# VIDILabs/instantvnr

Measured on AMD Instinct MI355X. Metric: fps at 1024^2 on 1024^3 volume, higher is better.
Workload: dtype f16

## Files before the change

### instantvnr_amd/csrc/grid_device.h

```cpp
#pragma once

#include "network.h"

namespace vnr {

typedef _Float16 half_t;
typedef _Float16 half2_t __attribute__((ext_vector_type(2)));
typedef _Float16 half4_t __attribute__((ext_vector_type(4)));
typedef _Float16 half8_t __attribute__((ext_vector_type(8)));
typedef float float2_t __attribute__((ext_vector_type(2)));
typedef float float4_t __attribute__((ext_vector_type(4)));
typedef float float8_t __attribute__((ext_vector_type(8)));
typedef float f32x16 __attribute__((ext_vector_type(16)));
typedef uint32_t uint4_t __attribute__((ext_vector_type(4)));

struct CornerSetup {
  float w[3];
  uint32_t g[3];
};

__device__ __forceinline__ CornerSetup level_setup(const LevelInfo& lv, uint32_t interpolation, float x, float y, float z)
{
  CornerSetup c;
  const float in[3] = {x, y, z};
#pragma unroll
  for (int d = 0; d < 3; ++d) {
    float p = __builtin_fmaf(in[d], lv.scale, 0.5f);
    const float t = __builtin_floorf(p);
    c.g[d] = (uint32_t)(int32_t)t;
    p -= t;
    c.w[d] = p;
  }
  if (interpolation == 1) {
    asm volatile("" ::: "memory");
#pragma unroll
    for (int d = 0; d < 3; ++d) c.w[d] = c.w[d] * c.w[d] * (3.0f - 2.0f * c.w[d]);
  }
  return c;
}

__device__ __forceinline__ uint32_t level_index(const LevelInfo& lv, uint32_t px, uint32_t py, uint32_t pz)
{
  if (lv.hashed == 1u) {
    return (px ^ (py * 2654435761u) ^ (pz * 805459861u)) & (lv.size - 1u);
  }
  if (lv.hashed >= 2u) {
    uint32_t idx = px;
    if (lv.hashed >= 3u) idx += py * lv.resolution;
    if (lv.hashed >= 4u) idx += pz * (lv.resolution * lv.resolution);
    return idx % lv.size;
  }
  uint32_t idx = px + py * lv.resolution + pz * (lv.resolution * lv.resolution);
  if (idx >= lv.size) {
    idx -= lv.size;
    if (idx >= lv.size) idx %= lv.size;
  }
  return idx;
}

__device__ __forceinline__ float corner_weight(const CornerSetup& c, int corner)
{
  const float wx = (corner & 1) ? c.w[0] : 1.0f - c.w[0];
  const float wy = (corner & 2) ? c.w[1] : 1.0f - c.w[1];
  const float wz = (corner & 4) ? c.w[2] : 1.0f - c.w[2];
  return (wx * wy) * wz;
}

template <int F> struct FeatVec;
template <> struct FeatVec<1> { typedef half_t type; };
template <> struct FeatVec<2> { typedef half2_t type; };
template <> struct FeatVec<4> { typedef half4_t type; };
template <> struct FeatVec<8> { typedef half8_t type; };

template <int F>
__device__ __forceinline__ void encode_level(const LevelInfo& lv, uint32_t interpolation, const half_t* __restrict__ table,
                                             float x, float y, float z, half_t* out)
{
  typedef typename FeatVec<F>::type vec_t;
  const CornerSetup c = level_setup(lv, interpolation, x, y, z);
  const vec_t* __restrict__ base = (const vec_t*)(table + (size_t)lv.offset * F);
  vec_t v[8];
#pragma unroll
  for (int corner = 0; corner < 8; ++corner) {
    const uint32_t idx = level_index(lv, c.g[0] + (corner & 1), c.g[1] + ((corner >> 1) & 1), c.g[2] + ((corner >> 2) & 1));
    v[corner] = base[idx];
  }
  half_t acc[F];
#pragma unroll
  for (int f = 0; f < F; ++f) acc[f] = (half_t)0.0f;
#pragma unroll
  for (int corner = 0; corner < 8; ++corner) {
    const float w = corner_weight(c, corner);
    const half_t* d = (const half_t*)&v[corner];
#pragma unroll
    for (int f = 0; f < F; ++f) {
      float prod = w * (float)d[f];
      if (F == 1) asm volatile("" : "+v"(prod));
      acc[f] = acc[f] + (half_t)prod;
    }
  }
#pragma unroll
  for (int f = 0; f < F; ++f) out[f] = acc[f];
}

typedef __amdgpu_buffer_rsrc_t table_rsrc_t;

#ifndef VNR_HASH_QUAD
#define VNR_HASH_QUAD 1
#endif

__device__ __forceinline__ table_rsrc_t make_table_rsrc(const void* base, uint32_t bytes)
{
  return __builtin_amdgcn_make_buffer_rsrc(const_cast<void*>(base), 0, (int)bytes, 0x00020000);
}

template <int F> struct RawFeat;
template <> struct RawFeat<1> {
  typedef unsigned short raw_t;
  static __device__ __forceinline__ raw_t load(table_rsrc_t r, uint32_t voff, uint32_t soff) { return __builtin_amdgcn_raw_buffer_load_b16(r, voff, soff, 0); }
};
template <> struct RawFeat<2> {
  typedef uint32_t raw_t;
  static __device__ __forceinline__ raw_t load(table_rsrc_t r, uint32_t voff, uint32_t soff) { return __builtin_amdgcn_raw_buffer_load_b32(r, voff, soff, 0); }
};
template <> struct RawFeat<4> {
  typedef uint32_t raw_t __attribute__((ext_vector_type(2)));
  static __device__ __forceinline__ raw_t load(table_rsrc_t r, uint32_t voff, uint32_t soff) { return __builtin_amdgcn_raw_buffer_load_b64(r, voff, soff, 0); }
};
template <> struct RawFeat<8> {
  typedef uint4_t raw_t;
  static __device__ __forceinline__ raw_t load(table_rsrc_t r, uint32_t voff, uint32_t soff) { return __builtin_amdgcn_raw_buffer_load_b128(r, voff, soff, 0); }
};

template <int F> struct PairFeat { static constexpr bool enabled = false; };
template <> struct PairFeat<2> {
  static constexpr bool enabled = true;
  typedef uint32_t pair_t __attribute__((ext_vector_type(2)));
  static __device__ __forceinline__ pair_t load(table_rsrc_t r, uint32_t voff, uint32_t soff) { return __builtin_amdgcn_raw_buffer_load_b64(r, voff, soff, 0); }
  static __device__ __forceinline__ uint32_t lo(pair_t p) { return p.x; }
  static __device__ __forceinline__ uint32_t hi(pair_t p) { return p.y; }
};
template <> struct PairFeat<4> {
  static constexpr bool enabled = true;
  typedef uint4_t pair_t;
  typedef uint32_t half_pair_t __attribute__((ext_vector_type(2)));
  static __device__ __forceinline__ pair_t load(table_rsrc_t r, uint32_t voff, uint32_t soff) { return __builtin_amdgcn_raw_buffer_load_b128(r, voff, soff, 0); }
  static __device__ __forceinline__ half_pair_t lo(pair_t p) { return half_pair_t{p.x, p.y}; }
  static __device__ __forceinline__ half_pair_t hi(pair_t p) { return half_pair_t{p.z, p.w}; }
};

typedef uint32_t uint8x32_t __attribute__((ext_vector_type(8)));
__device__ __noinline__ uint8x32_t level_indices_exact(const LevelInfo lv, uint32_t g0, uint32_t g1, uint32_t g2)
{
  uint8x32_t idx;
#pragma unroll
  for (int corner = 0; corner < 8; ++corner)
    idx[corner] = level_index(lv, g0 + (corner & 1), g1 + ((corner >> 1) & 1), g2 + ((corner >> 2) & 1));
  return idx;
}

template <int F, bool GENERAL = false>
__device__ __forceinline__ void gather_corners(const LevelInfo& lv, const CornerSetup& c, table_rsrc_t rsrc,
                                               typename RawFeat<F>::raw_t (&v)[8])
{
  constexpr uint32_t kBytes = (uint32_t)(F * 2);
  const uint32_t soff = lv.offset * kBytes;
  if (GENERAL && lv.hashed >= 2u) {
    const uint8x32_t idx = level_indices_exact(lv, c.g[0], c.g[1], c.g[2]);
#pragma unroll
    for (int corner = 0; corner < 8; ++corner) v[corner] = RawFeat<F>::load(rsrc, idx[corner] * kBytes, soff);
  } else if (lv.hashed) {
    const uint32_t mask = lv.size - 1u;
    const uint32_t hy0 = c.g[1] * 2654435761u, hy1 = hy0 + 2654435761u;
    const uint32_t hz0 = c.g[2] * 805459861u, hz1 = hz0 + 805459861u;
    const uint32_t x0 = c.g[0], x1 = c.g[0] + 1u;
    const uint32_t yz[4] = {hy0 ^ hz0, hy1 ^ hz0, hy0 ^ hz1, hy1 ^ hz1};
    constexpr uint32_t kGroupMask = (F == 2 && VNR_HASH_QUAD) ? 3u : PairFeat<F>::enabled ? 1u : 0u;
    if (kGroupMask && mask < kGroupMask) {
      const uint8x32_t idx = level_indices_exact(lv, c.g[0], c.g[1], c.g[2]);
#pragma unroll
      for (int corner = 0; corner < 8; ++corner) v[corner] = RawFeat<F>::load(rsrc, idx[corner] * kBytes, soff);
      return;
    }
#if VNR_HASH_QUAD
    if constexpr (F == 2) {
      const uint32_t m = (x0 & 1u) ? 3u : 1u;
      const bool far_x = (x0 & 3u) == 3u;
      uint32_t i1[4];
#pragma unroll
      for (int q = 0; q < 4; ++q) {
        const uint32_t i0 = (x0 ^ yz[q]) & mask;
        i1[q] = (x1 ^ yz[q]) & mask;
        const uint4_t g = __builtin_amdgcn_raw_buffer_load_b128(rsrc, (i0 & ~3u) * kBytes, soff, 0);
        const uint32_t k = i0 & 3u, k2 = k ^ m;
        const uint32_t a0 = (k & 1u) ? g.y : g.x, a1 = (k & 1u) ? g.w : g.z;
        const uint32_t b0 = (k & 1u) ? g.x : g.y, b1 = (k & 1u) ? g.z : g.w;
        v[2 * q] = (k & 2u) ? a1 : a0;
        v[2 * q + 1] = (k2 & 2u) ? b1 : b0;
      }
      if (far_x) {
#pragma unroll
        for (int q = 0; q < 4; ++q) v[2 * q + 1] = RawFeat<F>::load(rsrc, i1[q] * kBytes, soff);
      }
    } else
#endif
    if constexpr (PairFeat<F>::enabled) {
      const bool odd_x = (x0 & 1u) != 0u;
      uint32_t i1[4];
#pragma unroll
      for (int q = 0; q < 4; ++q) {
        const uint32_t i0 = (x0 ^ yz[q]) & mask;
        i1[q] = (x1 ^ yz[q]) & mask;
        const auto pr = PairFeat<F>::load(rsrc, (i0 & ~1u) * kBytes, soff);
        const bool up = (i0 & 1u) != 0u;
        v[2 * q] = up ? PairFeat<F>::hi(pr) : PairFeat<F>::lo(pr);
        v[2 * q + 1] = up ? PairFeat<F>::lo(pr) : PairFeat<F>::hi(pr);
      }
      if (odd_x) {
#pragma unroll
        for (int q = 0; q < 4; ++q) v[2 * q + 1] = RawFeat<F>::load(rsrc, i1[q] * kBytes, soff);
      }
    } else {
#pragma unroll
      for (int corner = 0; corner < 8; ++corner)
        v[corner] = RawFeat<F>::load(rsrc, ((((corner & 1) ? x1 : x0) ^ yz[corner >> 1]) & mask) * kBytes, soff);
    }
  } else {
    const uint32_t res = lv.resolution, res2 = lv.res2;
    const uint32_t base = c.g[0] + __umul24(c.g[1], res) + __umul24(c.g[2], res2);
    const bool bad = (c.g[0] > res) | (c.g[1] > res) | (c.g[2] > res) | (base + 1u + res + res2 >= lv.size);
    if (__builtin_amdgcn_ballot_w64(bad) != 0ull) {
      const uint8x32_t idx = level_indices_exact(lv, c.g[0], c.g[1], c.g[2]);
#pragma unroll
      for (int corner = 0; corner < 8; ++corner) v[corner] = RawFeat<F>::load(rsrc, idx[corner] * kBytes, soff);
    } else if constexpr (PairFeat<F>::enabled) {
#pragma unroll
      for (int q = 0; q < 4; ++q) {
        const uint32_t idx = base + ((q & 1) ? res : 0u) + ((q & 2) ? res2 : 0u);
        const auto pr = PairFeat<F>::load(rsrc, idx * kBytes, soff);
        v[2 * q] = PairFeat<F>::lo(pr);
        v[2 * q + 1] = PairFeat<F>::hi(pr);
      }
    } else {
#pragma unroll
      for (int corner = 0; corner < 8; ++corner) {
        const uint32_t idx = base + ((corner & 1) ? 1u : 0u) + ((corner & 2) ? res : 0u) + ((corner & 4) ? res2 : 0u);
        v[corner] = RawFeat<F>::load(rsrc, idx * kBytes, soff);
      }
    }
  }
}

template <int F>
__device__ __forceinline__ bool gather_corners_brick(const LevelInfo& lv, const CornerSetup& c, const uint8_t* __restrict__ image,
                                                     typename RawFeat<F>::raw_t (&v)[8])
{
  typedef typename RawFeat<F>::raw_t raw_t;
  if constexpr (F == 2) {
    typedef typename PairFeat<F>::pair_t pair_t;
    const uint32_t res = lv.resolution;
    const bool bad = (c.g[0] >= res) | (c.g[1] >= res) | (c.g[2] >= res);
    if (__builtin_amdgcn_ballot_w64(bad) != 0ull) return false;
    const uint32_t nbx = lv.pad1, nby = (res >> 1) + 1u;
    const uint32_t bx = (c.g[0] * 9363u) >> 16;
    const uint32_t wx = c.g[0] - 7u * bx, wy = c.g[1] & 1u, wz = c.g[2] & 1u;
    const uint32_t brick = __umul24(__umul24(c.g[2] >> 1, nby) + (c.g[1] >> 1), nbx) + bx;
    const uint32_t e0 = brick * 32u + ((wz << 4) | (wy << 3) | wx);
    const uint32_t dy = wy ? nbx * 32u - 8u : 8u;
    const uint32_t dz = wz ? nbx * nby * 32u - 16u : 16u;
    const uint8_t* base = image + (size_t)(lv.brick - 1u) * 128u;
#pragma unroll
    for (int q = 0; q < 4; ++q) {
      const uint32_t e = e0 + ((q & 1) ? dy : 0u) + ((q & 2) ? dz : 0u);
      const pair_t pr = *(const pair_t*)(base + (size_t)e * 4u);
      v[2 * q] = PairFeat<F>::lo(pr);
      v[2 * q + 1] = PairFeat<F>::hi(pr);
    }
    return true;
  }
  constexpr uint32_t LX = BrickShape<F>::lx, LY = BrickShape<F>::ly, LZ = BrickShape<F>::lz;
  constexpr uint32_t MX = (1u << LX) - 1u, MY = (1u << LY) - 1u, MZ = (1u << LZ) - 1u;
  constexpr uint32_t E = 1u << (LX + LY + LZ);
  constexpr uint32_t kBytes = (uint32_t)(F * 2);
  static_assert(E * kBytes == 128, "a brick is one 128-byte line");
  const uint32_t res = lv.resolution;
  const bool bad = (c.g[0] >= res) | (c.g[1] >= res) | (c.g[2] >= res);
  if (__builtin_amdgcn_ballot_w64(bad) != 0ull) return false;
  const uint32_t nbx = (res >> LX) + 1u, nby = (res >> LY) + 1u;
  const uint32_t wx = c.g[0] & MX, wy = c.g[1] & MY, wz = c.g[2] & MZ;
  const uint32_t brick = __umul24(__umul24(c.g[2] >> LZ, nby) + (c.g[1] >> LY), nbx) + (c.g[0] >> LX);
  const uint32_t e0 = brick * E + ((wz << (LX + LY)) | (wy << LX) | wx);
  const uint32_t dx = wx == MX ? E - MX : 1u;
  const uint32_t dy = wy == MY ? nbx * E - (MY << LX) : 1u << LX;
  const uint32_t dz = wz == MZ ? nbx * nby * E - (MZ << (LX + LY)) : 1u << (LX + LY);
  const uint8_t* base = image + (size_t)(lv.brick - 1u) * 128u;
  if constexpr (PairFeat<F>::enabled) {
    typedef typename PairFeat<F>::pair_t pair_t;
#pragma unroll
    for (int q = 0; q < 4; ++q) {
      const uint32_t e = e0 + ((q & 1) ? dy : 0u) + ((q & 2) ? dz : 0u);
      const pair_t pr = *(const pair_t*)(base + (size_t)e * kBytes);
      v[2 * q] = PairFeat<F>::lo(pr);
      v[2 * q + 1] = PairFeat<F>::hi(pr);
    }
    if (wx == MX) {
#pragma unroll
      for (int q = 0; q < 4; ++q) {
        const uint32_t e = e0 + ((q & 1) ? dy : 0u) + ((q & 2) ? dz : 0u) + dx;
        v[2 * q + 1] = *(const raw_t*)(base + (size_t)e * kBytes);
      }
    }
  } else {
#pragma unroll
    for (int corner = 0; corner < 8; ++corner) {
      const uint32_t e = e0 + ((corner & 1) ? dx : 0u) + ((corner & 2) ? dy : 0u) + ((corner & 4) ? dz : 0u);
      v[corner] = *(const raw_t*)(base + (size_t)e * kBytes);
    }
  }
  return true;
}

__device__ __forceinline__ half2_t weighted_pair(float w, uint32_t pair)
{
  float lo, hi;
  asm("v_fma_mix_f32 %0, %1, %2, 0 op_sel_hi:[1,0,0]" : "=v"(lo) : "v"(pair), "v"(w));
  asm("v_fma_mix_f32 %0, %1, %2, 0 op_sel:[1,0,0] op_sel_hi:[1,0,0]" : "=v"(hi) : "v"(pair), "v"(w));
  return __builtin_convertvector(float2_t{lo, hi}, half2_t);
}

template <int F>
__device__ __forceinline__ void blend_level(const float (&wd)[3], const typename FeatVec<F>::type (&v)[8], half_t* out)
{
  const float wx0 = 1.0f - wd[0], wx1 = wd[0], wy0 = 1.0f - wd[1], wy1 = wd[1], wz0 = 1.0f - wd[2], wz1 = wd[2];
  const float wxy[4] = {wx0 * wy0, wx1 * wy0, wx0 * wy1, wx1 * wy1};
  if constexpr (F == 1) {
    half_t acc = (half_t)0.0f;
#pragma unroll
    for (int corner = 0; corner < 8; ++corner) {
      float prod = (wxy[corner & 3] * ((corner & 4) ? wz1 : wz0)) * (float)v[corner];
      asm volatile("" : "+v"(prod));
      acc = acc + (half_t)prod;
    }
    out[0] = acc;
  } else {
    typedef uint32_t words_t __attribute__((ext_vector_type(F / 2)));
    half2_t acc[F / 2];
#pragma unroll
    for (int q = 0; q < F / 2; ++q) acc[q] = half2_t{(half_t)0.0f, (half_t)0.0f};
#pragma unroll
    for (int corner = 0; corner < 8; ++corner) {
      const float w = wxy[corner & 3] * ((corner & 4) ? wz1 : wz0);
      const words_t words = __builtin_bit_cast(words_t, v[corner]);
#pragma unroll
      for (int q = 0; q < F / 2; ++q) {
        uint32_t word;
        if constexpr (F == 2) word = __builtin_bit_cast(uint32_t, words); else word = words[q];
        acc[q] = acc[q] + weighted_pair(w, word);
      }
    }
#pragma unroll
    for (int q = 0; q < F / 2; ++q) { out[2 * q] = acc[q].x; out[2 * q + 1] = acc[q].y; }
  }
}

template <int F>
__device__ __forceinline__ typename RawFeat<F>::raw_t quantize_raw(typename RawFeat<F>::raw_t raw, float qt)
{
  typedef typename FeatVec<F>::type vec_t;
  vec_t v = __builtin_bit_cast(vec_t, raw);
  if constexpr (F == 1) {
    if (fabsf((float)v) < qt) v = (half_t)0.0f;
  } else {
#pragma unroll
    for (int f = 0; f < F; ++f) if (fabsf((float)v[f]) < qt) v[f] = (half_t)0.0f;
  }
  return __builtin_bit_cast(typename RawFeat<F>::raw_t, v);
}

template <int F, bool GENERAL = false>
__device__ __forceinline__ void encode_level_fast(const LevelInfo& lv, uint32_t interpolation, table_rsrc_t rsrc, const uint8_t* image,
                                                  float x, float y, float z, half_t* out, float quantize_threshold = 0.0f)
{
  typedef typename RawFeat<F>::raw_t raw_t;
  const CornerSetup c = level_setup(lv, interpolation, x, y, z);
  if (GENERAL && interpolation == 2u) {
    const raw_t one = RawFeat<F>::load(rsrc, level_index(lv, c.g[0], c.g[1], c.g[2]) * (uint32_t)(F * 2), lv.offset * (uint32_t)(F * 2));
    const typename FeatVec<F>::type vv = __builtin_bit_cast(typename FeatVec<F>::type, one);
    if constexpr (F == 1) out[0] = vv;
    else {
#pragma unroll
      for (int f = 0; f < F; ++f) out[f] = vv[f];
    }
    return;
  }
  raw_t v[8];
  if (lv.brick == 0u || !gather_corners_brick<F>(lv, c, image, v)) gather_corners<F, GENERAL>(lv, c, rsrc, v);
  if (GENERAL && quantize_threshold > 0.0f) {
#pragma unroll
    for (int corner = 0; corner < 8; ++corner) v[corner] = quantize_raw<F>(v[corner], quantize_threshold);
  }
  if constexpr (F >= 2) {
    typename FeatVec<F>::type vv[8];
#pragma unroll
    for (int corner = 0; corner < 8; ++corner) vv[corner] = __builtin_bit_cast(typename FeatVec<F>::type, v[corner]);
    blend_level<F>(c.w, vv, out);
    return;
  }
  const float wx0 = 1.0f - c.w[0], wx1 = c.w[0], wy0 = 1.0f - c.w[1], wy1 = c.w[1], wz0 = 1.0f - c.w[2], wz1 = c.w[2];
  const float wxy[4] = {wx0 * wy0, wx1 * wy0, wx0 * wy1, wx1 * wy1};
  half_t acc[F];
#pragma unroll
  for (int f = 0; f < F; ++f) acc[f] = (half_t)0.0f;
#pragma unroll
  for (int corner = 0; corner < 8; ++corner) {
    const float w = wxy[corner & 3] * ((corner & 4) ? wz1 : wz0);
    const half_t* d = (const half_t*)&v[corner];
#pragma unroll
    for (int f = 0; f < F; ++f) {
      float prod = w * (float)d[f];
      if (F == 1) asm volatile("" : "+v"(prod));
      acc[f] = acc[f] + (half_t)prod;
    }
  }
#pragma unroll
  for (int f = 0; f < F; ++f) out[f] = acc[f];
}

}
```

### instantvnr_amd/csrc/infer_kernel.h

```cpp
#pragma once
#include <algorithm>
#include <cstdlib>

#include "infer_tile.h"
#include "pack_rays.h"

namespace vnr {

struct FusedMlp {
  const uint16_t* packed;
  uint32_t lds_halves, width, n_hidden_matmuls, activation, output_activation;
  bool general;
  bool weights_global;
  float quantize_threshold;
};

struct InferArgs {
  const LevelInfo* levels;
  uint32_t n_levels, interpolation;
  const half_t* table;
  uint32_t table_bytes;
  const uint8_t* brick_image;
  const half_t* packed_mlp;
  const float* coords;
  float* out;
  half_t* features_out;
  half_t* acts_out;
  const uint32_t* n_ptr;
  const uint32_t* dest;
  uint32_t queue_mode;
  uint32_t out_stride;
  uint32_t n;
  uint32_t n_hidden_matmuls;
  uint32_t activation;
  uint32_t output_activation;
  uint32_t lds_halves;
  uint32_t sharers;
  uint32_t weights_global;
  float quantize_threshold;
  PackArgs pack;
};

template <int F, int K_IN, int W, int MODE, bool GENERAL>
__global__ void __launch_bounds__(64 * MlpShape<W>::WAVES) fused_infer_kernel(const InferArgs args)
{
  constexpr int NCHUNK = K_IN / 8;
  constexpr uint32_t WAVES = MlpShape<W>::WAVES;
  extern __shared__ __attribute__((aligned(16))) half_t lds[];

  const uint32_t lane = threadIdx.x & 63u;
  const uint32_t wave = threadIdx.x >> 6;

  if (MODE == 0 && WAVES == 4 && args.pack.n_blocks) {
    uint32_t* s_part = (uint32_t*)lds;
    for (uint32_t item = blockIdx.x; item < args.pack.n_blocks; item += gridDim.x) {
      pack_rays_block<4>(args.pack, item, s_part);
      __syncthreads();
    }
  }
  const uint32_t n = args.n_ptr ? min(*args.n_ptr, args.n) : args.n;
  const uint32_t n_tiles = (n + 63u) >> 6;
  const uint32_t xcd = blockIdx.x & 7u;
  const uint32_t per_xcd = (n_tiles + 7u) >> 3;
  const uint32_t waves_per_xcd = (gridDim.x >> 3) * WAVES;
  const uint32_t tile_end = min(n_tiles, (xcd + 1u) * per_xcd);
  if (xcd * per_xcd + (blockIdx.x >> 3) * WAVES >= tile_end) return;

  constexpr bool CAN_GLOBAL = GENERAL;
  const bool wglobal = CAN_GLOBAL && args.weights_global != 0u;
  if (MODE != 1 && !wglobal) {
    const uint4_t* src = (const uint4_t*)args.packed_mlp;
    uint4_t* dst = (uint4_t*)lds;
    for (uint32_t i = threadIdx.x; i < args.lds_halves / 8; i += blockDim.x) dst[i] = src[i];
    __syncthreads();
  }
  const uint32_t nh = args.n_hidden_matmuls;
  const uint32_t act = args.activation;
  const uint32_t h = lane >> 5;
  const uint32_t r = lane & 31u;
  const table_rsrc_t rsrc = make_table_rsrc(args.table, args.table_bytes);

  for (uint32_t tile = xcd * per_xcd + (blockIdx.x >> 3) * WAVES + wave; tile < tile_end; tile += waves_per_xcd) {
    const uint32_t i = tile * 64u + lane;
    const uint32_t ic = min(i, n - 1u);
    float3_packed p;
    uint32_t out_index = i;
    if (args.queue_mode) {
      const uint4_t rec = ((const uint4_t*)args.coords)[ic];
      p = {__uint_as_float(rec.x), __uint_as_float(rec.y), __uint_as_float(rec.z)};
      out_index = rec.w * args.out_stride;
    } else {
      p = ((const float3_packed*)args.coords)[ic];
      if (args.dest) out_index = args.dest[ic];
    }

    half8_t feat[NCHUNK];
    encode_tile<F, K_IN, GENERAL>(args.levels, args.n_levels, args.interpolation, rsrc, args.brick_image, p.x, p.y, p.z, feat,
                                  GENERAL ? args.quantize_threshold : 0.0f);

    if (MODE != 0 && args.features_out && i < n) {
      half8_t* dst = (half8_t*)(args.features_out + (size_t)i * K_IN);
#pragma unroll
      for (int c = 0; c < NCHUNK; ++c) dst[c] = feat[c];
    }
    if (MODE == 1) continue;

    float y;
    if (CAN_GLOBAL && wglobal)
      y = mlp_tile<W, K_IN, MODE == 2, GENERAL>(args.packed_mlp, feat, nh, act, h, r, args.acts_out, n, tile * 64u);
    else
      y = mlp_tile<W, K_IN, MODE == 2, GENERAL>((const half_t*)lds, feat, nh, act, h, r, args.acts_out, n, tile * 64u);
    if (i < n) args.out[out_index] = finish_output<GENERAL>(y, args.output_activation);
  }
}

template <int F, int K_IN, int W, int MODE, bool GENERAL>
static void launch_one(const InferArgs& a, size_t n_max, hipStream_t s)
{
  constexpr uint32_t WAVES = MlpShape<W>::WAVES;
  const Runtime& rt = Runtime::get();
  const uint32_t n_tiles = div_round_up(n_max, 64);
  uint32_t blocks = div_round_up(n_tiles, WAVES);
  static const uint32_t forced = [] {
    const char* e = std::getenv("VNR_AMD_INFER_BLOCKS_PER_CU");
    const int v = e ? std::atoi(e) : 0;
    return (uint32_t)(v >= 1 && v <= 64 ? v : 0);
  }();
  const size_t shmem = (MODE == 1 || a.weights_global) ? 16 : (size_t)a.lds_halves * sizeof(uint16_t);
  const uint32_t fit = (uint32_t)std::max<size_t>(1, std::min<size_t>(4, (160 * 1024) / std::max<size_t>(shmem, 1)));
  uint32_t max_blocks = (uint32_t)rt.n_cus * (forced ? forced : std::min(fit, a.sharers >= 2 ? 3u : 4u));
  if (!forced && a.n_ptr && a.queue_mode) max_blocks = std::min((uint32_t)rt.n_cus * 32u, std::max((uint32_t)rt.n_cus * 4u, n_tiles / 33u));
  if (blocks > max_blocks) blocks = max_blocks;
  blocks = next_multiple(blocks, 8);
  auto kernel = fused_infer_kernel<F, K_IN, W, MODE, GENERAL>;
  static bool attr_set = false;
  if (!attr_set) {
    VNR_HIP_CHECK(hipFuncSetAttribute((const void*)kernel, hipFuncAttributeMaxDynamicSharedMemorySize, 160 * 1024));
    attr_set = true;
  }
  kernel<<<blocks, 64 * WAVES, shmem, s>>>(a);
  VNR_HIP_CHECK(hipGetLastError());
}

template <int W, int MODE, bool GENERAL>
static void dispatch(uint32_t F, uint32_t K_IN, const InferArgs& a, size_t n_max, hipStream_t s)
{
#define VNR_CASE(f, k) if (F == f && K_IN == k) return launch_one<f, k, W, MODE, GENERAL>(a, n_max, s)
  VNR_CASE(1, 16); VNR_CASE(1, 32);
  VNR_CASE(2, 16); VNR_CASE(2, 32); VNR_CASE(2, 48); VNR_CASE(2, 64);
  VNR_CASE(4, 16); VNR_CASE(4, 32); VNR_CASE(4, 48); VNR_CASE(4, 64); VNR_CASE(4, 80); VNR_CASE(4, 96); VNR_CASE(4, 112); VNR_CASE(4, 128);
  VNR_CASE(8, 16); VNR_CASE(8, 32); VNR_CASE(8, 48); VNR_CASE(8, 64); VNR_CASE(8, 80); VNR_CASE(8, 96); VNR_CASE(8, 112); VNR_CASE(8, 128);
#undef VNR_CASE
  throw std::runtime_error("unsupported encoding shape: n_features_per_level=" + std::to_string(F) +
                           " padded width=" + std::to_string(K_IN));
}

#define VNR_DEFINE_FUSED_WIDTH(W, GENERAL, SUFFIX)                                                                        \
  void launch_fused_w##W##SUFFIX(int mode, uint32_t F, uint32_t K_IN, const InferArgs& a, size_t n_max, hipStream_t s)    \
  {                                                                                                                       \
    if (mode == 0) dispatch<W, 0, GENERAL>(F, K_IN, a, n_max, s);                                                         \
    else dispatch<W, 2, GENERAL>(F, K_IN, a, n_max, s);                                                                   \
  }

}
```

### instantvnr_amd/csrc/infer_tile.h

```cpp
#pragma once
#include "grid_device.h"

namespace vnr {

struct float3_packed { float x, y, z; };

template <int W> struct MlpShape {
  static_assert(W == 16 || W == 32 || W == 64 || W == 128, "FullyFusedMLP widths");
  static constexpr int MT = W >= 32 ? W / 32 : 1;
  static constexpr int RW = 32 * MT;
  static constexpr int KS = W / 16;
  static constexpr int STEP = 16 * RW;
  static constexpr int HIDDEN = KS * STEP;
  static constexpr int LAST = KS * 16;
  static constexpr int WAVES = W == 128 ? 8 : 4;
};
__host__ __device__ inline uint32_t mlp_rows_padded(uint32_t W) { return W >= 32u ? W : 32u; }
__host__ __device__ inline uint32_t packed_mlp_halves(uint32_t in_width, uint32_t W, uint32_t n_hidden_matmuls)
{
  const uint32_t step = 16u * mlp_rows_padded(W);
  return (in_width / 16u) * step + n_hidden_matmuls * (W / 16u) * step + (W / 16u) * 16u;
}

__host__ __device__ inline uint32_t packedT_halves(uint32_t in_width, uint32_t W, uint32_t nh)
{
  const uint32_t ks = W / 16u;
  return ks * 16u + nh * ks * 16u * mlp_rows_padded(W) + ks * 16u * (((in_width + 31u) / 32u) * 32u);
}

enum : uint32_t { kActNone = 0, kActReLU = 1, kActExponential = 2, kActSigmoid = 3, kActSquareplus = 4, kActSoftplus = 5 };

__device__ __forceinline__ float act_forward_f32(float x, uint32_t act)
{
  switch (act) {
  case kActExponential: return __expf(x);
  case kActSigmoid: return 1.0f / (1.0f + __expf(-x));
  case kActSquareplus: { const float t = x * 10.0f; return 0.5f * (t + sqrtf(t * t + 4.0f)) / 10.0f; }
  case kActSoftplus: return logf(expf(x * 10.0f) + 1.0f) / 10.0f;
  default: return x;
  }
}
__device__ __forceinline__ half_t act_forward_f16(half_t v, uint32_t act)
{
  if (act == kActNone) return v;
  if (act == kActReLU) return (__builtin_bit_cast(unsigned short, v) & 0x8000u) ? (half_t)0.0f : v;
  return (half_t)act_forward_f32((float)v, act);
}
__device__ __forceinline__ half_t act_backward_f16(half_t d, half_t y, uint32_t act)
{
  switch (act) {
  case kActReLU: return y > (half_t)0.0f ? d : (half_t)0.0f;
  case kActExponential: return d * y;
  case kActSigmoid: return d * (half_t)(y * (half_t)(1.0f - (float)y));
  case kActSquareplus: { const float t = (float)y * 10.0f; return d * (half_t)(t * t / (t * t + 1.0f)); }
  case kActSoftplus: return d * (half_t)(1.0f - __expf(-(float)y * 10.0f));
  default: return d;
  }
}

__device__ __noinline__ half8_t act_general8(half8_t r, uint32_t act)
{
#pragma unroll
  for (int j = 0; j < 8; ++j) r[j] = (half_t)act_forward_f32((float)r[j], act);
  return r;
}

template <bool GENERAL>
__device__ __forceinline__ half8_t pack_act(const f32x16& acc, int sh, uint32_t act)
{
  float8_t v;
#pragma unroll
  for (int j = 0; j < 8; ++j) v[j] = acc[8 * sh + j];
  half8_t r = __builtin_convertvector(v, half8_t);
  if (act == kActReLU) {
    const half8_t zero = {0, 0, 0, 0, 0, 0, 0, 0};
    r = __builtin_elementwise_max(r, zero);
  } else if (GENERAL && act > kActReLU) {
    r = act_general8(r, act);
  }
  return r;
}

__device__ __forceinline__ void swap_halves(uint32_t& a, uint32_t& b)
{
  const auto r = __builtin_amdgcn_permlane32_swap(a, b, false, false);
  a = r[0];
  b = r[1];
}

__device__ __forceinline__ void swap_halves8(half8_t& p, half8_t& q)
{
  uint4_t a = __builtin_bit_cast(uint4_t, p), b = __builtin_bit_cast(uint4_t, q);
#pragma unroll
  for (int i = 0; i < 4; ++i) {
    uint32_t x = a[i], y = b[i];
    swap_halves(x, y);
    a[i] = x;
    b[i] = y;
  }
  p = __builtin_bit_cast(half8_t, a);
  q = __builtin_bit_cast(half8_t, b);
}

template <int KS>
__device__ __forceinline__ void store_acts(half_t* row, const half8_t (&bf)[KS], uint32_t h)
{
#pragma unroll
  for (int s = 0; s < KS; ++s) {
    *(half4_t*)(row + 16 * s + 4 * h) = half4_t{bf[s][0], bf[s][1], bf[s][2], bf[s][3]};
    *(half4_t*)(row + 16 * s + 8 + 4 * h) = half4_t{bf[s][4], bf[s][5], bf[s][6], bf[s][7]};
  }
}

template <int W, int S1, bool TRAIN, bool GENERAL>
__device__ __forceinline__ float mlp_column_tile(const half_t* __restrict__ wgt, const half8_t (&b1)[S1], uint32_t nh, uint32_t act,
                                                 uint32_t h, uint32_t r, half_t* acts_out, size_t n, uint32_t smp, bool smp_ok)
{
  typedef MlpShape<W> Sh;
  constexpr int MT = Sh::MT, RW = Sh::RW, KS = Sh::KS;
  f32x16 acc[MT];
#pragma unroll
  for (int m = 0; m < MT; ++m)
#pragma unroll
    for (int e = 0; e < 16; ++e) acc[m][e] = 0.0f;
#pragma unroll
  for (int s = 0; s < S1; ++s) {
#pragma unroll
    for (int m = 0; m < MT; ++m) {
      const half8_t a = *(const half8_t*)(wgt + ((s * 2 + h) * RW + m * 32 + r) * 8);
      acc[m] = __builtin_amdgcn_mfma_f32_32x32x16_f16(a, b1[s], acc[m], 0, 0, 0);
    }
  }
  half8_t bf[KS];
#pragma unroll
  for (int s = 0; s < KS; ++s) bf[s] = pack_act<GENERAL>(acc[s >> 1], s & 1, act);
  if (TRAIN && acts_out && smp_ok) store_acts<KS>(acts_out + (size_t)smp * W, bf, h);

  for (uint32_t layer = 0; layer < nh; ++layer) {
    const half_t* w = wgt + S1 * Sh::STEP + layer * Sh::HIDDEN;
#pragma unroll
    for (int m = 0; m < MT; ++m)
#pragma unroll
      for (int e = 0; e < 16; ++e) acc[m][e] = 0.0f;
#pragma unroll
    for (int s = 0; s < KS; ++s) {
#pragma unroll
      for (int m = 0; m < MT; ++m) {
        const half8_t a = *(const half8_t*)(w + ((s * 2 + h) * RW + m * 32 + r) * 8);
        acc[m] = __builtin_amdgcn_mfma_f32_32x32x16_f16(a, bf[s], acc[m], 0, 0, 0);
      }
    }
#pragma unroll
    for (int s = 0; s < KS; ++s) bf[s] = pack_act<GENERAL>(acc[s >> 1], s & 1, act);
    if (TRAIN && acts_out && smp_ok) store_acts<KS>(acts_out + ((size_t)(layer + 1) * n + smp) * W, bf, h);
  }

  const half_t* wl = wgt + S1 * Sh::STEP + nh * Sh::HIDDEN;
  float part = 0.0f;
#pragma unroll
  for (int s = 0; s < KS; ++s) {
    const half8_t wv = *(const half8_t*)(wl + (s * 2 + h) * 8);
#pragma unroll
    for (int q = 0; q < 4; ++q) {
      const half2_t a2 = {bf[s][2 * q], bf[s][2 * q + 1]};
      const half2_t w2 = {wv[2 * q], wv[2 * q + 1]};
      part = __builtin_amdgcn_fdot2(a2, w2, part, false);
    }
  }
  return part;
}



template <int F, int K_IN, bool GENERAL = false>
__device__ __forceinline__ void encode_tile(const LevelInfo* levels, uint32_t n_levels, uint32_t interpolation, const table_rsrc_t& rsrc,
                                            const uint8_t* brick_image, float x, float y, float z, half8_t (&feat)[K_IN / 8],
                                            float quantize_threshold = 0.0f)
{
  constexpr int L_PAD = K_IN / F;
  typedef const __attribute__((address_space(4))) LevelInfo* const_levels_t;
  const LevelInfo* lvtab_generic = levels;
  asm volatile("" : "+s"(lvtab_generic));
  const const_levels_t lvtab = (const_levels_t)lvtab_generic;
  auto level_consts = [&](int l) {
    LevelInfo lv;
    lv.scale = __builtin_bit_cast(float, __builtin_amdgcn_readfirstlane(__builtin_bit_cast(int, lvtab[l].scale)));
    lv.resolution = __builtin_amdgcn_readfirstlane(lvtab[l].resolution);
    lv.res2 = __builtin_amdgcn_readfirstlane(lvtab[l].res2);
    lv.size = __builtin_amdgcn_readfirstlane(lvtab[l].size);
    lv.offset = __builtin_amdgcn_readfirstlane(lvtab[l].offset);
    lv.hashed = __builtin_amdgcn_readfirstlane(lvtab[l].hashed);
    lv.brick = __builtin_amdgcn_readfirstlane(lvtab[l].brick);
    lv.pad1 = __builtin_amdgcn_readfirstlane(lvtab[l].pad1);
    return lv;
  };
#pragma unroll
  for (int l = 0; l < L_PAD; ++l) {
    half_t o[F];
#pragma unroll
    for (int f = 0; f < F; ++f) o[f] = (half_t)0.0f;
    if (l < (int)n_levels) encode_level_fast<F, GENERAL>(level_consts(l), interpolation, rsrc, brick_image, x, y, z, o, quantize_threshold);
#pragma unroll
    for (int f = 0; f < F; ++f) feat[(l * F + f) / 8][(l * F + f) % 8] = o[f];
    if ((l & 3) == 3) __builtin_amdgcn_sched_barrier(0);
  }
}

template <int W, int K_IN, bool TRAIN, bool GENERAL = false>
__device__ __forceinline__ float mlp_tile(const half_t* __restrict__ wgt, half8_t (&feat)[K_IN / 8], uint32_t nh, uint32_t act, uint32_t h,
                                          uint32_t r, half_t* acts_out, size_t n, uint32_t tile_base)
{
  constexpr int S1 = K_IN / 16;
#pragma unroll
  for (int s = 0; s < S1; ++s) swap_halves8(feat[2 * s], feat[2 * s + 1]);

  float part[2];
#pragma unroll
  for (int nt = 0; nt < 2; ++nt) {
    half8_t b1[S1];
#pragma unroll
    for (int s = 0; s < S1; ++s) b1[s] = feat[2 * s + nt];
    const uint32_t smp = tile_base + 32u * nt + r;
    part[nt] = mlp_column_tile<W, S1, TRAIN, GENERAL>(wgt, b1, nh, act, h, r, acts_out, n, smp, smp < n);
  }

  uint32_t p0 = __builtin_bit_cast(uint32_t, part[0]), p1 = __builtin_bit_cast(uint32_t, part[1]);
  swap_halves(p0, p1);
  return __builtin_bit_cast(float, p0) + __builtin_bit_cast(float, p1);
}

template <bool GENERAL = false>
__device__ __forceinline__ float finish_output(float y, uint32_t out_act)
{
  if (!GENERAL) return (float)(half_t)y;
  return (float)act_forward_f16((half_t)y, out_act);
}

struct TileNet {
  const LevelInfo* levels;
  uint32_t n_levels, interpolation;
  const half_t* table;
  uint32_t table_bytes;
  const uint8_t* brick_image;
  const half_t* packed_mlp;
  uint32_t lds_halves, n_hidden_matmuls, activation, output_activation;
  uint32_t n_features, in_width, width;
  uint32_t general;
  float quantize_threshold;
};

template <int F, int K_IN, int W, bool GENERAL>
__device__ __forceinline__ float eval_tile(const TileNet& net, const half_t* __restrict__ lds, const table_rsrc_t& rsrc, float x, float y, float z)
{
  const uint32_t lane = threadIdx.x & 63u;
  half8_t feat[K_IN / 8];
  encode_tile<F, K_IN, GENERAL>(net.levels, net.n_levels, net.interpolation, rsrc, net.brick_image, x, y, z, feat, GENERAL ? net.quantize_threshold : 0.0f);
  const float v = mlp_tile<W, K_IN, false, GENERAL>(lds, feat, net.n_hidden_matmuls, net.activation, lane >> 5, lane & 31u, nullptr, 0, 0);
  return finish_output<GENERAL>(v, net.output_activation);
}

}
```

Measured before the change: 274.6.

## Overlap weight staging, record loads, and level-constant loads with gather work

Replaces the blocking copy of MLP weights into LDS with asynchronous global_load_lds DMA requests that are retired only before the first MLP use, so the copy overlaps the first tile's grid encoding. It also software-pipelines the per-tile coordinate record load one iteration ahead, and prefetches each level's constants with explicit s_load_dwordx8 issued right after the current level's corner gathers. The goal is to hide memory latency behind the encoding work. In exchange it adds hand-written inline asm (m0 juggling, lgkmcnt waits) that may constrain the compiler's scheduling, and it issues one out-of-range-clamped extra record load per wave.

```diff
diff --git a/instantvnr_amd/csrc/grid_device.h b/instantvnr_amd/csrc/grid_device.h
--- a/instantvnr_amd/csrc/grid_device.h
+++ b/instantvnr_amd/csrc/grid_device.h
@@ -377,15 +377,19 @@
   return __builtin_bit_cast(typename RawFeat<F>::raw_t, v);
 }
 
-template <int F, bool GENERAL = false>
+template <int F, bool GENERAL = false, class Issued>
 __device__ __forceinline__ void encode_level_fast(const LevelInfo& lv, uint32_t interpolation, table_rsrc_t rsrc, const uint8_t* image,
-                                                  float x, float y, float z, half_t* out, float quantize_threshold = 0.0f)
+                                                  float x, float y, float z, half_t* out, float quantize_threshold, Issued&& gathers_issued)
 {
   typedef typename RawFeat<F>::raw_t raw_t;
   const CornerSetup c = level_setup(lv, interpolation, x, y, z);
-  if (GENERAL && interpolation == 2u) {
-    const raw_t one = RawFeat<F>::load(rsrc, level_index(lv, c.g[0], c.g[1], c.g[2]) * (uint32_t)(F * 2), lv.offset * (uint32_t)(F * 2));
-    const typename FeatVec<F>::type vv = __builtin_bit_cast(typename FeatVec<F>::type, one);
+  const bool nearest = GENERAL && interpolation == 2u;
+  raw_t v[8];
+  if (nearest) v[0] = RawFeat<F>::load(rsrc, level_index(lv, c.g[0], c.g[1], c.g[2]) * (uint32_t)(F * 2), lv.offset * (uint32_t)(F * 2));
+  else if (lv.brick == 0u || !gather_corners_brick<F>(lv, c, image, v)) gather_corners<F, GENERAL>(lv, c, rsrc, v);
+  gathers_issued();
+  if (nearest) {
+    const typename FeatVec<F>::type vv = __builtin_bit_cast(typename FeatVec<F>::type, v[0]);
     if constexpr (F == 1) out[0] = vv;
     else {
 #pragma unroll
@@ -393,8 +397,6 @@
     }
     return;
   }
-  raw_t v[8];
-  if (lv.brick == 0u || !gather_corners_brick<F>(lv, c, image, v)) gather_corners<F, GENERAL>(lv, c, rsrc, v);
   if (GENERAL && quantize_threshold > 0.0f) {
 #pragma unroll
     for (int corner = 0; corner < 8; ++corner) v[corner] = quantize_raw<F>(v[corner], quantize_threshold);
@@ -426,4 +428,11 @@
   for (int f = 0; f < F; ++f) out[f] = acc[f];
 }
 
-}
+template <int F, bool GENERAL = false>
+__device__ __forceinline__ void encode_level_fast(const LevelInfo& lv, uint32_t interpolation, table_rsrc_t rsrc, const uint8_t* image,
+                                                  float x, float y, float z, half_t* out, float quantize_threshold = 0.0f)
+{
+  encode_level_fast<F, GENERAL>(lv, interpolation, rsrc, image, x, y, z, out, quantize_threshold, [] {});
+}
+
+}
diff --git a/instantvnr_amd/csrc/infer_kernel.h b/instantvnr_amd/csrc/infer_kernel.h
--- a/instantvnr_amd/csrc/infer_kernel.h
+++ b/instantvnr_amd/csrc/infer_kernel.h
@@ -41,6 +41,46 @@
   PackArgs pack;
 };
 
+#ifndef VNR_SCHED_STAGE
+#define VNR_SCHED_STAGE 1
+#endif
+#ifndef VNR_SCHED_RECORD
+#define VNR_SCHED_RECORD 1
+#endif
+
+__device__ __forceinline__ void load_pieces_to_lds(const uint4_t* src, uint32_t lds_base)
+{
+  uint32_t keep;
+  asm volatile("s_mov_b32 %0, m0\n\ts_mov_b32 m0, %2\n\ts_nop 0\n\tglobal_load_lds_dwordx4 %1, off\n\ts_mov_b32 m0, %0"
+               : "=&s"(keep) : "v"(src), "s"(lds_base) : "memory");
+}
+
+constexpr uint32_t kLdsDmaReach = 65536u / 16u;
+template <uint32_t WAVES>
+__device__ __forceinline__ void request_weights(const half_t* image, uint32_t n16, half_t* lds, uint32_t wave, uint32_t lane)
+{
+  const uint4_t* src = (const uint4_t*)image;
+  const uint32_t lds0 = (uint32_t)(uintptr_t)(__attribute__((address_space(3))) half_t*)lds;
+  const uint32_t n_dma = min(n16, kLdsDmaReach);
+  for (uint32_t c = __builtin_amdgcn_readfirstlane(wave) * 64u; c < n_dma; c += WAVES * 64u)
+    if (c + lane < n_dma) load_pieces_to_lds(src + c + lane, lds0 + c * 16u);
+  uint4_t* dst = (uint4_t*)lds;
+  for (uint32_t i0 = kLdsDmaReach + threadIdx.x; i0 < n16; i0 += 4u * 64u * WAVES) {
+    uint4_t v[4];
+#pragma unroll
+    for (uint32_t k = 0; k < 4; ++k) v[k] = src[min(i0 + k * 64u * WAVES, n16 - 1u)];
+#pragma unroll
+    for (uint32_t k = 0; k < 4; ++k)
+      if (i0 + k * 64u * WAVES < n16) dst[i0 + k * 64u * WAVES] = v[k];
+  }
+}
+
+__device__ __forceinline__ void retire_weights()
+{
+  asm volatile("s_waitcnt vmcnt(0)" ::: "memory");
+  __syncthreads();
+}
+
 template <int F, int K_IN, int W, int MODE, bool GENERAL>
 __global__ void __launch_bounds__(64 * MlpShape<W>::WAVES) fused_infer_kernel(const InferArgs args)
 {
@@ -68,31 +108,46 @@
 
   constexpr bool CAN_GLOBAL = GENERAL;
   const bool wglobal = CAN_GLOBAL && args.weights_global != 0u;
-  if (MODE != 1 && !wglobal) {
+  const bool stage = MODE != 1 && !wglobal;
+#if VNR_SCHED_STAGE
+  if (stage) request_weights<WAVES>(args.packed_mlp, args.lds_halves / 8, lds, wave, lane);
+  bool staged = !stage;
+#else
+  if (stage) {
     const uint4_t* src = (const uint4_t*)args.packed_mlp;
     uint4_t* dst = (uint4_t*)lds;
     for (uint32_t i = threadIdx.x; i < args.lds_halves / 8; i += blockDim.x) dst[i] = src[i];
     __syncthreads();
   }
+#endif
   const uint32_t nh = args.n_hidden_matmuls;
   const uint32_t act = args.activation;
   const uint32_t h = lane >> 5;
   const uint32_t r = lane & 31u;
   const table_rsrc_t rsrc = make_table_rsrc(args.table, args.table_bytes);
 
-  for (uint32_t tile = xcd * per_xcd + (blockIdx.x >> 3) * WAVES + wave; tile < tile_end; tile += waves_per_xcd) {
+  auto load_record = [&](uint32_t tile) {
     const uint32_t i = tile * 64u + lane;
     const uint32_t ic = min(i, n - 1u);
-    float3_packed p;
-    uint32_t out_index = i;
-    if (args.queue_mode) {
-      const uint4_t rec = ((const uint4_t*)args.coords)[ic];
-      p = {__uint_as_float(rec.x), __uint_as_float(rec.y), __uint_as_float(rec.z)};
-      out_index = rec.w * args.out_stride;
-    } else {
-      p = ((const float3_packed*)args.coords)[ic];
-      if (args.dest) out_index = args.dest[ic];
-    }
+    if (args.queue_mode) return ((const uint4_t*)args.coords)[ic];
+    const float3_packed p = ((const float3_packed*)args.coords)[ic];
+    return uint4_t{__float_as_uint(p.x), __float_as_uint(p.y), __float_as_uint(p.z), args.dest ? args.dest[ic] : i};
+  };
+  const uint32_t tile0 = xcd * per_xcd + (blockIdx.x >> 3) * WAVES + wave;
+#if VNR_SCHED_RECORD
+  uint4_t rec_next = load_record(tile0);
+#endif
+
+  for (uint32_t tile = tile0; tile < tile_end; tile += waves_per_xcd) {
+    const uint32_t i = tile * 64u + lane;
+#if VNR_SCHED_RECORD
+    const uint4_t rec = rec_next;
+    rec_next = load_record(tile + waves_per_xcd);
+#else
+    const uint4_t rec = load_record(tile);
+#endif
+    const float3_packed p = {__uint_as_float(rec.x), __uint_as_float(rec.y), __uint_as_float(rec.z)};
+    const uint32_t out_index = args.queue_mode ? rec.w * args.out_stride : rec.w;
 
     half8_t feat[NCHUNK];
     encode_tile<F, K_IN, GENERAL>(args.levels, args.n_levels, args.interpolation, rsrc, args.brick_image, p.x, p.y, p.z, feat,
@@ -105,6 +160,12 @@
     }
     if (MODE == 1) continue;
 
+#if VNR_SCHED_STAGE
+    if (!staged) {
+      retire_weights();
+      staged = true;
+    }
+#endif
     float y;
     if (CAN_GLOBAL && wglobal)
       y = mlp_tile<W, K_IN, MODE == 2, GENERAL>(args.packed_mlp, feat, nh, act, h, r, args.acts_out, n, tile * 64u);
@@ -112,6 +173,9 @@
       y = mlp_tile<W, K_IN, MODE == 2, GENERAL>((const half_t*)lds, feat, nh, act, h, r, args.acts_out, n, tile * 64u);
     if (i < n) args.out[out_index] = finish_output<GENERAL>(y, args.output_activation);
   }
+#if VNR_SCHED_STAGE
+  if (!staged) retire_weights();
+#endif
 }
 
 template <int F, int K_IN, int W, int MODE, bool GENERAL>
diff --git a/instantvnr_amd/csrc/infer_tile.h b/instantvnr_amd/csrc/infer_tile.h
--- a/instantvnr_amd/csrc/infer_tile.h
+++ b/instantvnr_amd/csrc/infer_tile.h
@@ -1,5 +1,12 @@
 #pragma once
+#include <type_traits>
+#include <utility>
+
 #include "grid_device.h"
+
+#ifndef VNR_SCHED_LEVELS
+#define VNR_SCHED_LEVELS 1
+#endif
 
 namespace vnr {
 
@@ -172,6 +179,12 @@
 
 
 
+template <class Fn, int... I>
+__device__ __forceinline__ void static_for(std::integer_sequence<int, I...>, Fn&& fn)
+{
+  (fn(std::integral_constant<int, I>{}), ...);
+}
+
 template <int F, int K_IN, bool GENERAL = false>
 __device__ __forceinline__ void encode_tile(const LevelInfo* levels, uint32_t n_levels, uint32_t interpolation, const table_rsrc_t& rsrc,
                                             const uint8_t* brick_image, float x, float y, float z, half8_t (&feat)[K_IN / 8],
@@ -182,6 +195,49 @@
   const LevelInfo* lvtab_generic = levels;
   asm volatile("" : "+s"(lvtab_generic));
   const const_levels_t lvtab = (const_levels_t)lvtab_generic;
+#if VNR_SCHED_LEVELS
+  typedef uint32_t level_raw_t __attribute__((ext_vector_type(8)));
+  static_assert(sizeof(LevelInfo) == 32 && L_PAD <= kMaxLevels, "one s_load_dwordx8 per level, inside the table");
+  auto level_request = [&](auto level) {
+    level_raw_t raw;
+    asm volatile("s_load_dwordx8 %0, %1, %2" : "=s"(raw) : "s"(lvtab), "n"(decltype(level)::value * 32) : "memory");
+    return raw;
+  };
+  auto level_wait = [](level_raw_t& raw) { asm volatile("s_waitcnt lgkmcnt(0)" : "+s"(raw)); };
+  auto level_unpack = [](const level_raw_t& raw) {
+    LevelInfo lv;
+    lv.scale = __builtin_bit_cast(float, raw[0]);
+    lv.resolution = raw[1];
+    lv.res2 = raw[2];
+    lv.size = raw[3];
+    lv.offset = raw[4];
+    lv.hashed = raw[5];
+    lv.brick = raw[6];
+    lv.pad1 = raw[7];
+    return lv;
+  };
+  level_raw_t raw[2];
+  raw[0] = level_request(std::integral_constant<int, 0>{});
+  level_wait(raw[0]);
+  static_for(std::make_integer_sequence<int, L_PAD>{}, [&](auto level) {
+    constexpr int l = decltype(level)::value;
+    half_t o[F];
+#pragma unroll
+    for (int f = 0; f < F; ++f) o[f] = (half_t)0.0f;
+    if (l < (int)n_levels) {
+      encode_level_fast<F, GENERAL>(level_unpack(raw[l & 1]), interpolation, rsrc, brick_image, x, y, z, o, quantize_threshold, [&] {
+        if constexpr (l + 1 < L_PAD) {
+          raw[(l + 1) & 1] = level_request(std::integral_constant<int, l + 1>{});
+          __builtin_amdgcn_sched_barrier(0);
+        }
+      });
+      if constexpr (l + 1 < L_PAD) level_wait(raw[(l + 1) & 1]);
+    }
+#pragma unroll
+    for (int f = 0; f < F; ++f) feat[(l * F + f) / 8][(l * F + f) % 8] = o[f];
+    if ((l & 3) == 3) __builtin_amdgcn_sched_barrier(0);
+  });
+#else
   auto level_consts = [&](int l) {
     LevelInfo lv;
     lv.scale = __builtin_bit_cast(float, __builtin_amdgcn_readfirstlane(__builtin_bit_cast(int, lvtab[l].scale)));
@@ -204,6 +260,7 @@
     for (int f = 0; f < F; ++f) feat[(l * F + f) / 8][(l * F + f) % 8] = o[f];
     if ((l & 3) == 3) __builtin_amdgcn_sched_barrier(0);
   }
+#endif
 }
 
 template <int W, int K_IN, bool TRAIN, bool GENERAL = false>
```

Result: no change. 273.6 (-0.4%).
